# oharari/Convex-Combination-of-Gaussian-Processes

Hardware: AMD Instinct MI355X
Metric: GP log-lik evals/sec (n x n fp64, batched over hyperpar grid) (higher is better)
Workload: dtype f64; 1 GPU; cfg4: synthetic maximin-LHS 5-D design n=4096, K=3 anisotropic components, 512-point hyperparameter grid sharded over the GPUs; n=4096, d=5, K=3, evals_total=512, evals_per_gpu=512, parallelism=grid sharded over 1 GPU(s), one all-gather

## Files before the change

### convex-combination-of-gaussian-processes_amd/api.py

```python
from __future__ import annotations

import ctypes
from ctypes import POINTER, c_char_p, c_double, c_int, c_size_t, c_void_p

import numpy as np

from ._lib import load_library

MEAN_PROFILE_BETA = 0
MEAN_ZERO_PLUS_TAU2 = 1
PRIOR_INVGAMMA, PRIOR_GV, PRIOR_ISO, PRIOR_ANI = 0, 1, 2, 3
T_COV, T_UPDATE, T_DIAG, T_TRSM, T_SOLVE, T_FUSED = range(6)
KERNEL_GAUSS, KERNEL_MATERN, KERNEL_MATERN_SPLINE = 0, 1, 2
OPT_FUSE_DIAG, OPT_TAIL_STRIPS, OPT_WIDE_OFFSETS, OPT_SMALL_GRID16 = 2, 3, 4, 5
OPT_SCHED, OPT_SCHED_POLICY, OPT_PREDICT_FACTOR = 7, 8, 9
TIMING_NAMES = ("cov", "update", "diag", "trsm", "solve", "fused", "sweep")

_dp = POINTER(c_double)
_ip = POINTER(c_int)

SIGNATURES = {
    "ccgp_create": (c_int, [c_int, POINTER(c_void_p)]),
    "ccgp_destroy": (c_int, [c_void_p]),
    "ccgp_last_error": (c_char_p, [c_void_p]),
    "ccgp_version": (c_char_p, []),
    "ccgp_set_stream": (c_int, [c_void_p, c_void_p]),
    "ccgp_set_kernel": (c_int, [c_void_p, c_int, c_double]),
    "ccgp_set_workspace_limit": (c_int, [c_void_p, c_size_t]),
    "ccgp_set_option": (c_int, [c_void_p, c_int, c_int]),
    "ccgp_reserve": (c_int, [c_void_p, c_int, c_int, c_int, c_int, c_int]),
    "ccgp_synchronize": (c_int, [c_void_p]),
    "ccgp_corr_matrix": (c_int, [c_void_p, _dp, c_int, c_int, _dp, _dp]),
    "ccgp_corr_cross": (c_int, [c_void_p, _dp, c_int, _dp, c_int, c_int, _dp, _dp]),
    "ccgp_mixed_corr_matrix": (c_int, [c_void_p, _dp, c_int, c_int, c_int, _dp, _dp]),
    "ccgp_mixed_corr_cross": (c_int, [c_void_p, _dp, c_int, _dp, c_int, c_int, c_int, _dp, _dp]),
    "ccgp_beta_mle": (c_int, [c_void_p, _dp, _dp, c_int, _dp]),
    "ccgp_sigma2_mle": (c_int, [c_void_p, _dp, _dp, c_int, c_double, _dp]),
    "ccgp_loglik_batch": (c_int, [c_void_p, _dp, c_int, c_int, _dp, c_int, _dp, c_int, c_double,
                                  c_int, c_double, _dp, _dp, _ip]),
    "ccgp_loglik_batch_dev": (c_int, [c_void_p, c_void_p, c_int, c_int, c_void_p, c_int, c_void_p,
                                      c_int, c_double, c_int, c_double, c_void_p, c_void_p, c_void_p]),
    "ccgp_loglik_grad_batch": (c_int, [c_void_p, _dp, c_int, c_int, _dp, c_int, _dp, c_int, c_double,
                                       _dp, _dp, _dp, _ip]),
    "ccgp_logpost": (c_int, [c_void_p, _dp, c_int, c_int, _dp, c_double, c_int, _dp, _dp, _dp, _dp,
                             _dp, _dp, _ip]),
    "ccgp_logpost_batch": (c_int, [c_void_p, _dp, c_int, c_int, _dp, c_double, c_int, _dp, c_int, _dp, _dp, _dp, _dp, _ip]),
    "ccgp_grid_marginal": (c_int, [c_void_p, _dp, c_int, c_int, _dp, c_double, _dp, c_int, c_int,
                                   c_double, c_int, c_double, _dp, _ip, _dp]),
# ... 552 lines not shown
```

### convex-combination-of-gaussian-processes_amd/csrc/blocked.hip

```cpp
#include <cstdlib>
#include <vector>

#include "ccgp_internal.h"
#include "sched_logic.h"

namespace ccgp {

typedef double d4 __attribute__((ext_vector_type(4)));

namespace {

__device__ __forceinline__ int tid_now() {
  int t = threadIdx.x;
  asm volatile("" : "+v"(t));
  return t;
}

__device__ __forceinline__ constexpr int swz_src(int l, int parity) { return (((l >> 3) ^ parity) << 4) + ((l & 7) << 1); }

struct GemmArgs {
  double* A;
  size_t a_stride;
  int npad;
  double* invd;
  size_t invd_stride;
  int j, nt, nb;
  int ld;
  int ne;
  int extra_lower;
  int mode;
  double* E;
  size_t e_stride;
  int lde;
  int rows_only;
  int fuse_diag;
  int tail_strips;
  int wide;
  int n_s1;
  int tail_s;
  double* logdet_part;
  int* status;
  int n;
  double ptol;
};

template <int S, bool THIN>
struct TileGeom {
  static constexpr int CW = kTile / S;
  static constexpr int NX = THIN ? (S == 1 ? 2 : 1) : (S == 1 ? 4 : 2);
  static constexpr int NY = THIN ? 1 : (S == 4 ? 2 : 4);
  static constexpr int BK = 16;
  __device__ static int row0(int wave) { return THIN ? 0 : (S == 4 ? wave * 32 : (wave >> 1) * 64); }
  __device__ static int col0(int wave) {
    return THIN ? wave * NX * 16 : (S == 4 ? 0 : (wave & 1) * (S == 1 ? 64 : 32));
  }
};

template <int S, bool THIN, bool TRI>
__device__ __forceinline__ int col_block(int wave, int x) {
  if constexpr (TRI && !THIN) return (wave & 1) + 2 * x;
  else return (TileGeom<S, THIN>::col0(wave) >> 4) + x;
}

template <bool IL>
struct AccMap {
  int row0, col0, l15, l4;
  __device__ __forceinline__ AccMap() {
    const int lane = tid_now() & 63, wave = tid_now() >> 6;
    row0 = TileGeom<1, false>::row0(wave); col0 = TileGeom<1, false>::col0(wave); l15 = lane & 15; l4 = lane >> 4;
  }
  __device__ __forceinline__ int row(int y) const { return IL ? row0 + 4 * l15 + y : row0 + 16 * y + l15; }
  __device__ __forceinline__ int col(int x, int r) const { return IL ? col0 + 16 * r + 4 * l4 + x : col0 + 16 * x + l4 + 4 * r; }
  static constexpr __device__ __forceinline__ int dcol(int x, int r) { return IL ? 16 * r + x : 16 * x + 4 * r; }
  __device__ __forceinline__ double* lane_base(double* C, int ld) const {
    return IL ? C + row0 + 4 * l15 + (size_t)(col0 + 4 * l4) * ld : C + row0 + l15 + (size_t)(col0 + l4) * ld;
  }
};

template <int S, bool THIN, bool TRI = false>
__device__ __forceinline__ void gemm_accumulate(double* smem, const double* P, int ldP, const double* Q,
                                                int ldQ, int Kdim,
                                                d4 (&acc)[TileGeom<S, THIN>::NX][TileGeom<S, THIN>::NY]) {
  static_assert(!TRI || S == 1, "the triangular skip is only wired for full-width tiles");
  constexpr int CW = TileGeom<S, THIN>::CW;
  constexpr int NX = TileGeom<S, THIN>::NX;
  constexpr int NY = TileGeom<S, THIN>::NY;
  constexpr int BKs = TileGeom<S, THIN>::BK;
  constexpr int STAGE = BKs * kTile + BKs * CW;
  constexpr int CPI = kTile / CW;
  constexpr int QI = BKs / CPI / 4;
  const int tid = tid_now(), lane = tid & 63, wave = tid >> 6;
  const int row0 = TileGeom<S, THIN>::row0(wave);
  const int col0 = TileGeom<S, THIN>::col0(wave);
  const bool active = !THIN || col0 < CW;
  const int l15 = lane & 15, l4 = lane >> 4;

#pragma unroll
  for (int x = 0; x < NX; ++x)
#pragma unroll
    for (int y = 0; y < NY; ++y) acc[x][y] = d4{0.0, 0.0, 0.0, 0.0};

  const double* pP = P + swz_src(lane, wave & 1) + (size_t)wave * ldP;
  const size_t stepP = (size_t)4 * ldP;
  constexpr int LPC = 64 / CPI;
  const int qcol_in = lane / LPC, ql = lane % LPC;
  const int qpar = CPI == 1 ? (wave & 1) : (qcol_in & 1);
  const double* pQ = Q + swz_src(ql, qpar) + (size_t)(CPI * wave + qcol_in) * ldQ;
  const size_t stepQ = (size_t)(4 * CPI) * ldQ;

  auto issue = [&](int stage) {
    double* Ps_ = smem + stage * STAGE + wave * kTile;
    double* Qs_ = smem + stage * STAGE + BKs * kTile + wave * kTile;
#pragma unroll
    for (int q = 0; q < BKs / 4; ++q)
      __builtin_amdgcn_global_load_lds((const __attribute__((address_space(1))) void*)(pP + q * stepP),
                                       (__attribute__((address_space(3))) void*)(Ps_ + 4 * q * kTile), 16, 0, 0);
#pragma unroll
    for (int q = 0; q < QI; ++q)
      __builtin_amdgcn_global_load_lds((const __attribute__((address_space(1))) void*)(pQ + q * stepQ),
                                       (__attribute__((address_space(3))) void*)(Qs_ + 4 * q * kTile), 16, 0, 0);
    pP += (BKs / 4) * stepP;
    pQ += QI * stepQ;
  };

  static_assert(BKs == 16, "the pipeline below is written for four k-steps per stage");
  double pfA[NY], qfA[NX], pfB[NY], qfB[NX];
  const int sw = l4 & 1;
#define CCGP_LOADF(PF, QF, STG, KK)                                                              \
  do {                                                                                          \
    const double* Ps_ = smem + (STG) * STAGE;                                                   \
    const double* Qs_ = Ps_ + BKs * kTile;                                                      \
    _Pragma("unroll") for (int y = 0; y < NY; ++y)                                              \
        PF[y] = Ps_[((KK) * 4 + l4) * kTile + ((((row0 >> 4) + y) ^ sw) << 4) + l15];           \
    _Pragma("unroll") for (int x = 0; x < NX; ++x)                                              \
        QF[x] = Qs_[((KK) * 4 + l4) * CW + ((col_block<S, THIN, TRI>(wave, x) ^ sw) << 4) + l15]; \
    __builtin_amdgcn_sched_barrier(0);                                                          \
  } while (0)
#define CCGP_MFMAS(PF, QF, KT, X0, X1)                                                           \
  do {                                                                                          \
    if (active) {                                                                               \
      _Pragma("unroll") for (int x = (X0); x < (X1); ++x) {                                     \
        if (TRI && col_block<S, THIN, TRI>(wave, x) * 16 + 15 < (KT) * BKs) continue;           \
        _Pragma("unroll") for (int y = 0; y < NY; ++y)                                          \
            acc[x][y] = __builtin_amdgcn_mfma_f64_16x16x4f64(QF[x], PF[y], acc[x][y], 0, 0, 0); \
      }                                                                                         \
    }                                                                                           \
    __builtin_amdgcn_sched_barrier(0);                                                          \
  } while (0)
  constexpr int XH = NX > 1 ? 1 : NX;

  const int nk = Kdim / BKs;
  issue(0);
  __syncthreads();
  if (nk > 1) issue(1);
  CCGP_LOADF(pfA, qfA, 0, 0);
  for (int kt = 0; kt < nk; ++kt) {
    const int stg = kt & 1;
    CCGP_MFMAS(pfA, qfA, kt, 0, XH);
    CCGP_LOADF(pfB, qfB, stg, 1);
    CCGP_MFMAS(pfA, qfA, kt, XH, NX);
    CCGP_MFMAS(pfB, qfB, kt, 0, XH);
    CCGP_LOADF(pfA, qfA, stg, 2);
    CCGP_MFMAS(pfB, qfB, kt, XH, NX);
    CCGP_MFMAS(pfA, qfA, kt, 0, XH);
    CCGP_LOADF(pfB, qfB, stg, 3);
    CCGP_MFMAS(pfA, qfA, kt, XH, NX);
    if (kt + 1 < nk) {
      __syncthreads();
      if (kt + 2 < nk) issue(stg);
    }
    CCGP_MFMAS(pfB, qfB, kt, 0, XH);
    if (kt + 1 < nk) CCGP_LOADF(pfA, qfA, stg ^ 1, 0);
    CCGP_MFMAS(pfB, qfB, kt, XH, NX);
  }
#undef CCGP_LOADF
#undef CCGP_MFMAS
}



__device__ __forceinline__ bool fits_buffer_offsets(int Kdim, int ld) {
  return ((size_t)Kdim + 32) * (size_t)ld * 8 < 0xFFFF0000ull;
}

__device__ __forceinline__ void tile_accumulate_il(double* smem, const double* P, int ldP, const double* Q,
                                                   int ldQ, int Kdim, d4 (&acc)[4][4]) {
  constexpr int BKs = 16, STAGE = 2 * BKs * kTile;
  typedef double d2 __attribute__((ext_vector_type(2)));
  const int tid = tid_now(), lane = tid & 63;
  const int wave = __builtin_amdgcn_readfirstlane(tid >> 6);
  const int row0 = (wave >> 1) * 64, col0 = (wave & 1) * 64;
  const int l15 = lane & 15, l4 = lane >> 4;
#pragma unroll
  for (int x = 0; x < 4; ++x)
#pragma unroll
    for (int y = 0; y < 4; ++y) acc[x][y] = d4{0.0, 0.0, 0.0, 0.0};

  const __amdgpu_buffer_rsrc_t rP = __builtin_amdgcn_make_buffer_rsrc((void*)P, 0, -1, 0x00020000);
  const __amdgpu_buffer_rsrc_t rQ = __builtin_amdgcn_make_buffer_rsrc((void*)Q, 0, -1, 0x00020000);
  const unsigned lane_b = (unsigned)lane * 16;
  const unsigned stepP = (unsigned)ldP * 32, stepQ = (unsigned)ldQ * 32;
  unsigned oP = (unsigned)wave * (unsigned)ldP * 8, oQ = (unsigned)wave * (unsigned)ldQ * 8;
  auto request = [&](int stage, int r) {
    double* dst = smem + stage * STAGE + (r >> 2) * (BKs * kTile) + (wave + 4 * (r & 3)) * kTile;
    if (r < 4)
      __builtin_amdgcn_raw_ptr_buffer_load_lds(rP, (__attribute__((address_space(3))) void*)dst, 16, lane_b,
// ... 142 lines not shown
  } while (0)
#define CCGP_RMFMAS(PF, QF, X0, X1)                                                              \
  do {                                                                                          \
    _Pragma("unroll") for (int x = (X0); x < (X1); ++x)                                         \
      _Pragma("unroll") for (int y = 0; y < NY; ++y)                                            \
          acc[x][y] = __builtin_amdgcn_mfma_f64_16x16x4f64(QF[x], PF[y], acc[x][y], 0, 0, 0);   \
    __builtin_amdgcn_sched_barrier(0);                                                          \
  } while (0)

  const int nk = Kdim / BKd;
  const int pre = nk < NST ? nk : NST;
  for (int t = 0; t < pre; ++t) issue(t);
  __builtin_amdgcn_sched_barrier(0);
  wait_and_meet(pre - 1);
  CCGP_RLOADF(pfA, qfA, 0, 0);
  for (int kt = 0; kt < nk; ++kt) {
    const int slot = kt & (NST - 1);
    CCGP_RLOADF(pfB, qfB, slot, 1);
    CCGP_RMFMAS(pfA, qfA, 0, 2);
    if (kt + 1 < nk) {
      const int last_issued = kt + NST - 1 < nk - 1 ? kt + NST - 1 : nk - 1;
      wait_and_meet(last_issued - (kt + 1));
      if (kt + NST < nk) issue(slot);
      __builtin_amdgcn_sched_barrier(0);
    }
    CCGP_RMFMAS(pfB, qfB, 0, 1);
    if (kt + 1 < nk) CCGP_RLOADF(pfA, qfA, (kt + 1) & (NST - 1), 0);
    CCGP_RMFMAS(pfB, qfB, 1, 2);
  }
#undef CCGP_RLOADF
#undef CCGP_RMFMAS
}

template <int S, bool THIN, bool TRI = false, bool RING = false>
__device__ __forceinline__ void gemm_tile(double* smem, const double* P, int ldP, const double* Q,
                                          int ldQ, int Kdim, double* C, int ld, int mode) {
  constexpr int NX = TileGeom<S, THIN>::NX;
  constexpr int NY = TileGeom<S, THIN>::NY;
  d4 acc[NX][NY];
  if constexpr (RING) {
    static_assert((S == 2 || S == 4) && !THIN && !TRI, "the four-stage ring exists for half- and quarter-width update strips");
    strip_accumulate_ring<S>(smem, P, ldP, Q, ldQ, Kdim, acc);
  } else {
    gemm_accumulate<S, THIN, TRI>(smem, P, ldP, Q, ldQ, Kdim, acc);
  }
  const int lane = tid_now() & 63, wave = tid_now() >> 6;
  const int row0 = TileGeom<S, THIN>::row0(wave), col0 = TileGeom<S, THIN>::col0(wave);
  const int l15 = lane & 15, l4 = lane >> 4;
  if (THIN && col0 >= TileGeom<S, THIN>::CW) return;
#pragma unroll
  for (int x = 0; x < NX; ++x) {
    double cv[NY][4];
    if (mode == 0) {
#pragma unroll
      for (int y = 0; y < NY; ++y)
#pragma unroll
        for (int r = 0; r < 4; ++r)
          cv[y][r] = C[row0 + y * 16 + l15 + (size_t)(col_block<S, THIN, TRI>(wave, x) * 16 + l4 + 4 * r) * ld];
    }
#pragma unroll
    for (int y = 0; y < NY; ++y)
#pragma unroll
      for (int r = 0; r < 4; ++r) {
        double* p = C + row0 + y * 16 + l15 + (size_t)(col_block<S, THIN, TRI>(wave, x) * 16 + l4 + 4 * r) * ld;
        *p = mode == 0 ? cv[y][r] - acc[x][y][r] : acc[x][y][r];
      }
  }
}


template <int W>
__device__ __forceinline__ void diag_rhs_accumulate(double* smem, const double* Qp, const double* Tp, int ld,
                                                    int Kdim, d4 (&acc)[11]) {
  constexpr int BKs = 16, TR = 16, STAGE = BKs * kTile + BKs * TR;
  constexpr int RA = W, RB = 7 - W;
  constexpr int CBMAX = RA > RB ? RA : RB;
  constexpr bool XTRA = 2 * W + 1 > CBMAX;
  constexpr int NQ = CBMAX + 1 + (XTRA ? 2 : 0);
  constexpr int NR = W < 2 ? 5 : 4;
  auto frag_of = [](int cb) constexpr { return cb <= CBMAX ? cb : CBMAX + 1 + (cb - 2 * W); };
  auto cb_of_frag = [](int f) constexpr { return f <= CBMAX ? f : 2 * W + (f - CBMAX - 1); };
  const int lane = tid_now() & 63, l15 = lane & 15, l4 = lane >> 4, sw = l4 & 1;

  const __amdgpu_buffer_rsrc_t rQ = __builtin_amdgcn_make_buffer_rsrc((void*)Qp, 0, -1, 0x00020000);
  const __amdgpu_buffer_rsrc_t rT = __builtin_amdgcn_make_buffer_rsrc((void*)Tp, 0, -1, 0x00020000);
  const unsigned lane_q = (unsigned)(swz_src(lane, W & 1) * 8);
  const unsigned lane_t = (unsigned)((((lane & 7) << 1) + (size_t)(lane >> 3) * ld) * 8);
  const unsigned stepQ = (unsigned)ld * 32;
  unsigned oQ = (unsigned)W * (unsigned)ld * 8, oT = (unsigned)(8 * W) * (unsigned)ld * 8;
  auto request = [&](int stage, int r) {
    double* St_ = smem + stage * STAGE;
    if (r < 4)
      __builtin_amdgcn_raw_ptr_buffer_load_lds(rQ, (__attribute__((address_space(3))) void*)(St_ + (W + 4 * r) * kTile),
                                               16, lane_q, oQ + (unsigned)r * stepQ, 0, 0);
    else
      __builtin_amdgcn_raw_ptr_buffer_load_lds(rT, (__attribute__((address_space(3))) void*)(St_ + BKs * kTile + W * 8 * TR),
                                               16, lane_t, oT, 0, 0);
  };
  auto advance = [&]() { oQ += 4 * stepQ; oT += (unsigned)BKs * (unsigned)ld * 8; };

// ... 280 lines not shown
  for (int off = 32; off > 0; off >>= 1) lsum += __shfl_down(lsum, off, 64);
  if ((tid & 63) == 0) red[tid >> 6] = lsum;
  __syncthreads();
  if (tid == 0) {
    g.logdet_part[(size_t)b * g.nt + g.j] = bad ? kNaN : (red[0] + red[1] + red[2] + red[3]);
    if (bad && g.status[b] == 0) g.status[b] = g.j * kTile + bad;
  }

  double* W = g.invd + (size_t)b * g.invd_stride + (size_t)g.j * kTile * kTile;
#pragma unroll
  for (int bb = 0; bb < 8; ++bb) {
    const int c = tx + 16 * bb;
    const double dc = bad ? 1.0 : dvec[c];
    const double sq = sqrt(dc), rs = 1.0 / sq;
#pragma unroll
    for (int a = 0; a < 8; ++a) {
      const int r = ty + 16 * a;
      if (a >= bb) {
        double v = r > c ? M[a][bb] * rs : (r == c ? sq : 0.0);
        C[r + (size_t)c * ld] = bad ? kNaN : v;
      }
      double w = 0.0;
      if (bb >= a) w = c >= r ? I[a][bb] * rs : 0.0;
      W[c + (size_t)r * kTile] = bad ? kNaN : w;
    }
  }
}

__global__ __launch_bounds__(256) void diag_kernel(DiagArgs g) {
  __shared__ double lds[kDiagLdsDoubles];
  diag_factor(g, blockIdx.x, lds);
}

__host__ __device__ inline int gemm_units_per_matrix(int mode, int nt, int j, int ne, int S, int rows_only = 0) {
  if (rows_only) return mode == 0 ? ne * S : ne;
  return mode == 0 ? 1 + ((nt - 1 - j) + ne) * S : (nt - j) + ne;
}

template <int MODE, int S>
__device__ __forceinline__ void gemm_unit(const GemmArgs& g, double* smem, int j, int b, int i, int strip, bool ring) {
  const int ld = g.ld;
  double* Ab = g.A + (size_t)b * g.a_stride;
  const bool thin = i == g.nt;
  const int c0 = strip * (ring ? kTile / g.tail_s : kTile / S);

  int k0 = 0;
  if (g.extra_lower && i > g.nt) {
    const int te = i - g.nt - 1;
    if (j < te || (MODE == 0 && j == te)) return;
    k0 = te * kTile;
  }
  double* rowbase = Ab + (size_t)i * kTile;
  int rld = ld;
  if (g.E && i > g.nt) {
    rowbase = g.E + (size_t)b * g.e_stride + (size_t)(i - g.nt - 1) * kTile;
    rld = g.lde;
  }
  const double* P;
  const double* Q;
  int ldP, ldQ, Kdim;
  if (MODE == 0) {
    P = rowbase + (size_t)k0 * rld;
    Q = Ab + (size_t)j * kTile + c0 + (size_t)k0 * ld;
    ldP = rld;
    ldQ = ld;
    Kdim = j * kTile - k0;
  } else {
    P = rowbase + (size_t)j * kTile * rld;
    Q = g.invd + (size_t)b * g.invd_stride + (size_t)j * kTile * kTile + c0;
    ldP = rld;
    ldQ = kTile;
    Kdim = kTile;
  }
  double* C = rowbase + ((size_t)j * kTile + c0) * rld;
  constexpr bool TRI = MODE == 1 && S == 1;
  if constexpr (MODE == 1) {
    if (thin) { gemm_tile<S, true, TRI>(smem, P, ldP, Q, ldQ, Kdim, C, rld, MODE); return; }
  }
  if constexpr (MODE == 0 && S == 1) {
    if (ring) {
      if (g.tail_s == 4) gemm_tile<4, false, false, true>(smem, P, ldP, Q, ldQ, Kdim, C, rld, MODE);
      else gemm_tile<2, false, false, true>(smem, P, ldP, Q, ldQ, Kdim, C, rld, MODE);
      return;
    }
    if (!g.wide && fits_buffer_offsets(Kdim, ldP > ldQ ? ldP : ldQ)) {
      update_tile_il(smem, P, ldP, Q, ldQ, Kdim, C, rld);
      return;
    }
  }
  gemm_tile<S, false, TRI>(smem, P, ldP, Q, ldQ, Kdim, C, rld, MODE);
}

__device__ __forceinline__ void diag_unit(const GemmArgs& g, double* smem, int j, int b) {
  const int ld = g.ld;
  double* Ab = g.A + (size_t)b * g.a_stride;
  diag_rhs_tile(smem, Ab + (size_t)j * kTile, Ab + g.npad, ld, j * kTile,
                Ab + (size_t)j * kTile + (size_t)j * kTile * ld, Ab + g.npad + (size_t)j * kTile * ld, g.wide);
  if (g.fuse_diag) {
    __syncthreads();
    diag_factor(diag_args(g, j), b, smem);
  }
}

template <int MODE, int S>
__device__ __forceinline__ void gemm_dispatch(const GemmArgs& g, double* smem) {
  const int L = blockIdx.x;
  int b, i, strip = 0;
  bool ring = false;
  if (MODE == 0 && !g.rows_only) {
    const int nb8 = (g.nb + 7) & ~7;
    if (L < nb8) {
      if (L < g.nb) diag_unit(g, smem, g.j, L);
      return;
    }
    const int nfull = (g.nt - 1 - g.j) + g.ne;
    const int Lt = L - nb8;
    int u1;
    if (S == 1) {
      if (Lt >= g.n_s1) {
        const int q = Lt - g.n_s1;
        u1 = g.n_s1 + ((q / (8 * g.tail_s)) << 3) + (q & 7);
        strip = (q >> 3) % g.tail_s;
        ring = true;
      } else {
        u1 = Lt;
      }
    } else {
      u1 = ((Lt / (8 * S)) << 3) + (Lt & 7);
      strip = (Lt >> 3) % S;
    }
    const int per_grp = 8 * nfull;
    const int grp = u1 / per_grp, r = u1 % per_grp;
    b = grp * 8 + (r & 7);
    if (b >= g.nb) return;
    i = g.j + 1 + (r >> 3);
    if (i >= g.nt) i += 1;
  } else {
    const int per_grp = 8 * gemm_units_per_matrix(MODE, g.nt, g.j, g.ne, S, g.rows_only);
    const int grp = L / per_grp, r = L % per_grp;
    b = grp * 8 + (r & 7);
    if (b >= g.nb) return;
    const int u = r >> 3;
    if (g.rows_only) {
      strip = MODE == 0 ? u % S : 0;
      i = g.nt + 1 + (MODE == 0 ? u / S : u);
    } else {
      i = g.j + 1 + u;
    }
  }
  gemm_unit<MODE, S>(g, smem, g.j, b, i, strip, ring);
}

#define CCGP_DEFINE_GEMM(NAME, MODE, S, WPS)                                            \
  __global__ __launch_bounds__(256, WPS) void NAME(GemmArgs g) {                        \
    extern __shared__ __attribute__((aligned(16))) double smem[];                       \
    gemm_dispatch<MODE, S>(g, smem);                                                     \
  }
CCGP_DEFINE_GEMM(chol_update_kernel, 0, 1, 2)
CCGP_DEFINE_GEMM(chol_update_s2_kernel, 0, 2, 2)
CCGP_DEFINE_GEMM(chol_trsm_kernel, 1, 1, 2)
#undef CCGP_DEFINE_GEMM

#include "blocked_sched.inc"


static int update_tail(int nb8, int tiles, int quarters, int* ts) {
  const long w1 = (long)nb8 * (1 + tiles), all_tiles = (long)nb8 * tiles;
  const long rem = w1 % 256;
  *ts = 2;
  if (rem == 0 || all_tiles == 0) return 0;
  long tail = rem < all_tiles ? rem : all_tiles;
  if (tail != rem && w1 > 256) return 0;
  if (quarters && w1 > 256 && (rem - tail) + 4 * tail <= 512) { *ts = 4; return (int)tail; }
  if (rem + tail > 256) return 0;
  return (int)tail;
}

static void launch_gemm(hipStream_t s, GemmArgs g, int mode, int S) {
  const int nb8 = round_up(g.nb, 8);
  int units = nb8 * gemm_units_per_matrix(mode, g.nt, g.j, g.ne, S, g.rows_only);
  if (mode == 0 && !g.rows_only) {
    const int tiles = (g.nt - 1 - g.j) + g.ne;
    int ts = 2;
    const int tail = (S == 1 && g.tail_strips) ? update_tail(nb8, tiles, g.tail_strips == 1, &ts) : 0;
    g.n_s1 = nb8 * tiles - tail;
    g.tail_s = ts;
    units = nb8 + (S == 1 ? g.n_s1 + ts * tail : nb8 * tiles * S);
  }
  const dim3 grid(units), block(256);
  if (mode == 0) {
    if (S == 1) hipLaunchKernelGGL(chol_update_kernel, grid, block, gemm_lds_bytes<1>(), s, g);
    else hipLaunchKernelGGL(chol_update_s2_kernel, grid, block, gemm_lds_bytes<2>(), s, g);
  } else {
    hipLaunchKernelGGL(chol_trsm_kernel, grid, block, gemm_lds_bytes<1>(), s, g);
  }
}

struct RhsArgs {
  double* A;
  size_t a_stride;
  int npad, n;
  const double* y;
  int ld;
  int identity;
};

__global__ __launch_bounds__(256) void rhs_rows_kernel(RhsArgs g) {
  const int ld = g.ld;
  double* Ab = g.A + (size_t)blockIdx.y * g.a_stride;
  const int c = blockIdx.x * 16 + (threadIdx.x >> 4);
  const int r = threadIdx.x & 15;
  double v = 0.0;
  if (c < g.n) v = r == 0 ? g.y[c] : (r == 1 ? 1.0 : 0.0);
// ... 440 lines not shown

struct GroupRun {
  ccgp_handle* h;
  hipStream_t s;
  const double* X;
  int n, d;
  const double* y;
  DrawView dv;
  int b0, nb, npad, nt;
  double sigma2;
  int mean_mode;
  double tau2;
  BlockedWs w;
  double* loglik;
  double* beta;
  int* status;
  const BlockedJob* job;
  GemmArgs g{};
  void begin() {
    const BlockedJob* pr = job && job->kind == kJobPredict ? job : nullptr;
    nt = npad / kTile;
    {
      ScopedTimer t(h, CCGP_T_COV, s);
      launch_cov_tiles(s, X, n, d, dv, b0, nb, w.A, w.a_stride, npad, mean_mode, sigma2, tau2, w.ld, w.xpad, w.upad);
      RhsArgs ra{w.A, w.a_stride, npad, n, y, w.ld, job && job->kind >= kJobInverse ? 1 : 0};
      hipLaunchKernelGGL(rhs_rows_kernel, dim3(npad / 16, nb), dim3(256), 0, s, ra);
      if (pr)
        launch_cov_cross_batched(s, pr->Xtest, pr->m, X, n, d, dv, b0, nb, w.A + npad + kTile, w.a_stride,
                                 w.ld);
    }
    g.A = w.A; g.a_stride = w.a_stride; g.npad = npad; g.invd = w.invd;
    g.invd_stride = (size_t)nt * kTile * kTile; g.nt = nt; g.nb = nb; g.ld = w.ld; g.ne = w.ne;
    g.extra_lower = job && job->kind >= kJobInverse ? 1 : 0;
    g.fuse_diag = h->opt_fuse_diag; g.tail_strips = h->opt_tail_strips; g.wide = h->opt_wide_offsets; g.logdet_part = w.z; g.status = status + b0; g.n = n;
    g.ptol = pivot_tolerance(mean_mode, n);
  }

  void update(int j) {
    if (j == 0) return;
    ScopedTimer t(h, CCGP_T_UPDATE, s);
    g.j = j;
    g.mode = 0;
    launch_gemm(s, g, 0, 1);
  }

  void panel(int j) {
    if (j == 0 || !g.fuse_diag) {
      ScopedTimer t(h, CCGP_T_DIAG, s);
      hipLaunchKernelGGL(diag_kernel, dim3(nb), dim3(256), 0, s, diag_args(g, j));
    }
    {
      ScopedTimer t(h, CCGP_T_TRSM, s);
      g.j = j;
      g.mode = 1;
      launch_gemm(s, g, 1, 1);
    }
  }

  void finish() {
    const BlockedJob* pr = job && job->kind == kJobPredict ? job : nullptr;
    {
      ScopedTimer t(h, CCGP_T_SOLVE, s);
      FinishArgs fa{};
      fa.A = w.A; fa.a_stride = w.a_stride; fa.npad = npad; fa.logdet_part = w.z; fa.params = dv.params;
      fa.ldp = dv.ldp; fa.K = dv.K; fa.b0 = b0; fa.nt = nt; fa.n = n; fa.sigma2 = sigma2;
      fa.mode = mean_mode; fa.loglik = loglik; fa.beta = beta; fa.status = status; fa.ld = w.ld;
      fa.s11_out = w.fin; fa.beta_out = w.fin + nb;
// ... 151 lines not shown
```

### convex-combination-of-gaussian-processes_amd/csrc/capi.hip

```cpp
#include <algorithm>
#include <cmath>
#include <cstdio>
#include <cstdlib>
#include <cstring>
#include <exception>
#include <initializer_list>
#include <map>
#include <memory>
#include <new>
#include <vector>

#include "ccgp_internal.h"
#include "special_math.h"
#include "stage_layout.h"

using namespace ccgp;

namespace {

#define CCGP_HIP(call)                                                              \
  do {                                                                              \
    hipError_t e_ = (call);                                                         \
    if (e_ != hipSuccess) {                                                         \
      h->err = std::string(#call) + ": " + hipGetErrorString(e_);                   \
// ... 612 lines not shown

int ccgp_set_kernel(ccgp_handle* h, int family, double nu) try {
  if (!h) return CCGP_EINVAL;
  if (family == CCGP_KERNEL_GAUSS) {
    h->fam = ccgp::KernelFamily{};
    return CCGP_OK;
  }
  if ((family != CCGP_KERNEL_MATERN && family != CCGP_KERNEL_MATERN_SPLINE) || !(nu > 1.0) || !(nu <= 10.0))
    return fail(h, CCGP_EINVAL, "ccgp_set_kernel: family must be CCGP_KERNEL_GAUSS, or CCGP_KERNEL_MATERN / CCGP_KERNEL_MATERN_SPLINE with 1 < nu <= 10 (the range the quadrature is validated on; the scripts use 5)");
  h->fam.id = family;
  h->fam.nu = nu;
  h->fam.norm = 1.0 / (std::tgamma(nu) * std::pow(2.0, nu - 1.0));
  return CCGP_OK;
} CCGP_GUARD_END(h)

int ccgp_set_workspace_limit(ccgp_handle* h, size_t bytes) try {
  if (!h || bytes < (size_t(1) << 20)) return CCGP_EINVAL;
  h->ws_limit = bytes;
  return CCGP_OK;
} CCGP_GUARD_END(h)

int ccgp_set_option(ccgp_handle* h, int option, int value) try {
  if (!h) return CCGP_EINVAL;
  if (option == CCGP_OPT_TAIL_STRIPS && value >= 0 && value <= 2) {
    h->opt_tail_strips = value;
    return CCGP_OK;
  }
  if (option == CCGP_OPT_FUSE_DIAG && (value == 0 || value == 1)) {
    h->opt_fuse_diag = value;
    return CCGP_OK;
  }
  if (option == CCGP_OPT_WIDE_OFFSETS && (value == 0 || value == 1)) {
    h->opt_wide_offsets = value;
    return CCGP_OK;
  }
  if (option == CCGP_OPT_SMALL_GRID16 && (value == 0 || value == 1)) {
    h->opt_small_grid16 = value;
    return CCGP_OK;
  }
  if (option == CCGP_OPT_PREDICT_FACTOR && (value == 0 || value == 1)) {
    h->opt_predict_factor = value;
    return CCGP_OK;
  }
  if (option == CCGP_OPT_SCHED && value >= 0 && value <= 3) {
    h->opt_sched = value;
    return CCGP_OK;
  }
  if (option == CCGP_OPT_SCHED_POLICY && value >= 0 && value <= 31) {
    h->opt_sched_policy = value;
    return CCGP_OK;
  }
  return fail(h, CCGP_EINVAL, "ccgp_set_option: unknown option or value");
} CCGP_GUARD_END(h)

int ccgp_synchronize(ccgp_handle* h) try {
  if (!h) return CCGP_EINVAL;
  CCGP_HIP(hipStreamSynchronize(h->stream));
  return CCGP_OK;
} CCGP_GUARD_END(h)

int ccgp_reserve(ccgp_handle* h, int n, int d, int K, int B, int m) try {
  if (!h || bad_shape(n, d, K) || B < 1 || m < 0) return fail(h, CCGP_EINVAL, "ccgp_reserve: bad argument");
  CCGP_HIP(hipSetDevice(h->device));
  const bool gauss = h->fam.id == 0;
  const bool sweep_predict = m > 0 && small_route(Op::Predict, gauss, n, d, K) == Route::Blocked;
  if (sweep_predict || small_route(Op::Loglik, gauss, n, d, K) == Route::Blocked) {
// ... 931 lines not shown
```

### convex-combination-of-gaussian-processes_amd/csrc/ccgp_internal.h

```cpp
#pragma once

#include <hip/hip_runtime.h>

#include <cstddef>
#include <atomic>
#include <cstdint>
#include <mutex>
#include <string>
#include <vector>

#include "../../include/ccgp.h"
#include "exp_table.h"
#include "small_layout.h"

namespace ccgp {

constexpr int kTile = 128;

constexpr double kSolvePivotEps = 2.220446049250313e-16;
__host__ __device__ inline double pivot_tolerance(int mean_mode, int n) { return mean_mode == 0 ? n * kSolvePivotEps : 0.0; }

}

namespace ccgp {

struct TimedSpan {
  int id;
  hipEvent_t e0, e1;
};

struct KernelFamily {
  int id = 0;
  double nu = 0.0;
  double norm = 0.0;
};

}

namespace ccgp {
constexpr int kPullSlices = 4;
}

struct ccgp_handle {
  int device = 0;
  hipStream_t own_stream = nullptr;
  hipStream_t stream = nullptr;
  size_t ws_limit = size_t(24) << 30;
  int opt_small_grid16 = 0;
  int opt_predict_factor = 1;
  int opt_fuse_diag = 1;
  int opt_tail_strips = 1;
  int opt_wide_offsets = 0;
  int opt_sched = 3;
  int opt_sched_policy = 11;
  int sched_timeout_ms = 30000;
  int sched_backlog_min = 0;
  int n_cus = 256;
  unsigned long long* sched_prof_dev = nullptr;
  int sched_prof_wgs = 0;
  void* ws = nullptr;
  size_t ws_bytes = 0;
  void* stage = nullptr;
  size_t stage_bytes = 0;
  void* pin = nullptr;
  size_t pin_bytes = 0;
  size_t pin_in = 0;
  hipStream_t aux_stream = nullptr;
  hipEvent_t aux_fork = nullptr, aux_join = nullptr;
  hipEvent_t pull_ev[ccgp::kPullSlices] = {};
  std::string err;
  ccgp::KernelFamily fam;
  unsigned timing = 0;
  std::vector<ccgp::TimedSpan> spans;
  size_t spans_used = 0;
};

namespace ccgp {

struct DrawView {
  const double* params;
  int ldp;
  int K;
  int d;
  KernelFamily fam;
};
// ... 278 lines not shown
```

### include/ccgp.h

```cpp
#ifndef CCGP_H
#define CCGP_H

#include <stddef.h>
#include <stdint.h>

#ifdef __cplusplus
extern "C" {
#endif

typedef struct ccgp_handle ccgp_handle;

enum {
  CCGP_OK = 0,
  CCGP_EINVAL = -1,
  CCGP_EHIP = -2,
  CCGP_ENOMEM = -3,
  CCGP_EUNSUPPORTED = -4
};

enum {
  CCGP_MEAN_PROFILE_BETA = 0,
  CCGP_MEAN_ZERO_PLUS_TAU2 = 1
};

enum {
  CCGP_PRIOR_INVGAMMA = 0,
  CCGP_PRIOR_GV = 1,
  CCGP_PRIOR_ISO = 2,
  CCGP_PRIOR_ANI = 3
};

int ccgp_create(int device, ccgp_handle** out);
int ccgp_destroy(ccgp_handle* h);
const char* ccgp_last_error(const ccgp_handle* h);
const char* ccgp_version(void);
int ccgp_set_stream(ccgp_handle* h, void* hip_stream);
enum { CCGP_KERNEL_GAUSS = 0, CCGP_KERNEL_MATERN = 1, CCGP_KERNEL_MATERN_SPLINE = 2 };
int ccgp_set_kernel(ccgp_handle* h, int family, double nu);
int ccgp_set_workspace_limit(ccgp_handle* h, size_t bytes);
enum { CCGP_OPT_FUSE_DIAG = 2, CCGP_OPT_TAIL_STRIPS = 3, CCGP_OPT_WIDE_OFFSETS = 4, CCGP_OPT_SMALL_GRID16 = 5,
       CCGP_OPT_SCHED = 7, CCGP_OPT_SCHED_POLICY = 8, CCGP_OPT_PREDICT_FACTOR = 9 };
int ccgp_set_option(ccgp_handle* h, int option, int value);
int ccgp_reserve(ccgp_handle* h, int n, int d, int K, int B, int m);
int ccgp_synchronize(ccgp_handle* h);

int ccgp_corr_matrix(ccgp_handle* h, const double* X, int n, int d, const double* theta,
                     double* out_R);
int ccgp_corr_cross(ccgp_handle* h, const double* Xnew, int m, const double* X, int n, int d,
                    const double* theta, double* out);

int ccgp_mixed_corr_matrix(ccgp_handle* h, const double* X, int n, int d, int K,
                           const double* params, double* out_R);
int ccgp_mixed_corr_cross(ccgp_handle* h, const double* Xnew, int m, const double* X, int n,
                          int d, int K, const double* params, double* out);

int ccgp_beta_mle(ccgp_handle* h, const double* R_inv, const double* y, int n, double* out_beta);
int ccgp_sigma2_mle(ccgp_handle* h, const double* R_inv, const double* y, int n, double beta,
                    double* out_sigma2);

int ccgp_loglik_batch(ccgp_handle* h, const double* X, int n, int d, const double* y, int K,
                      const double* params, int B, double sigma2, int mean_mode, double tau2,
                      double* out_loglik, double* out_beta, int* status);
int ccgp_loglik_batch_dev(ccgp_handle* h, const double* dX, int n, int d, const double* dy, int K,
                          const double* dparams, int B, double sigma2, int mean_mode, double tau2,
                          double* d_loglik, double* d_beta, int* d_status);

int ccgp_loglik_grad_batch(ccgp_handle* h, const double* X, int n, int d, const double* y, int K,
                           const double* params, int B, double sigma2, double* out_loglik,
                           double* out_beta, double* out_grad, int* status);

int ccgp_logpost(ccgp_handle* h, const double* X, int n, int d, const double* y, double sigma2,
                 int prior_id, const double* theta_t, const double* prior_pars, double* out_val,
                 double* out_beta, double* out_loglik, double* out_Rinv, int* status);
int ccgp_logpost_batch(ccgp_handle* h, const double* X, int n, int d, const double* y, double sigma2, int prior_id,
// ... 91 lines not shown
```

Measured before the change: 2653 evals/s.

## Pair panel-solve tiles per workgroup, streaming two output tiles through one pipeline

In the blocked Cholesky panel solve (mode 1), each workgroup now handles two vertically adjacent output tiles instead of one. It streams their K-loops back to back through the same double-buffered LDS pipeline, storing the first tile at a seam callback and then resetting the accumulators. This halves the number of trsm workgroups, amortises pipeline fill/drain and the shared Q operand setup, and keeps the prefetch running across the tile boundary. In exchange there is less parallelism per launch, longer per-workgroup latency, and a new default-on option that changes the unit indexing.

```diff
diff --git a/convex-combination-of-gaussian-processes_amd/api.py b/convex-combination-of-gaussian-processes_amd/api.py
--- a/convex-combination-of-gaussian-processes_amd/api.py
+++ b/convex-combination-of-gaussian-processes_amd/api.py
@@ -13,7 +13,7 @@
 T_COV, T_UPDATE, T_DIAG, T_TRSM, T_SOLVE, T_FUSED = range(6)
 KERNEL_GAUSS, KERNEL_MATERN, KERNEL_MATERN_SPLINE = 0, 1, 2
 OPT_FUSE_DIAG, OPT_TAIL_STRIPS, OPT_WIDE_OFFSETS, OPT_SMALL_GRID16 = 2, 3, 4, 5
-OPT_SCHED, OPT_SCHED_POLICY, OPT_PREDICT_FACTOR = 7, 8, 9
+OPT_SCHED, OPT_SCHED_POLICY, OPT_PREDICT_FACTOR, OPT_TRSM_PAIR = 7, 8, 9, 10
 TIMING_NAMES = ("cov", "update", "diag", "trsm", "solve", "fused", "sweep")
 
 _dp = POINTER(c_double)
diff --git a/convex-combination-of-gaussian-processes_amd/csrc/blocked.hip b/convex-combination-of-gaussian-processes_amd/csrc/blocked.hip
--- a/convex-combination-of-gaussian-processes_amd/csrc/blocked.hip
+++ b/convex-combination-of-gaussian-processes_amd/csrc/blocked.hip
@@ -42,6 +42,7 @@
   int* status;
   int n;
   double ptol;
+  int trsm_pair;
 };
 
 template <int S, bool THIN>
@@ -77,11 +78,14 @@
   }
 };
 
-template <int S, bool THIN, bool TRI = false>
+struct NoSeam {};
+template <int S, bool THIN, bool TRI = false, class SEAM = NoSeam>
 __device__ __forceinline__ void gemm_accumulate(double* smem, const double* P, int ldP, const double* Q,
                                                 int ldQ, int Kdim,
-                                                d4 (&acc)[TileGeom<S, THIN>::NX][TileGeom<S, THIN>::NY]) {
+                                                d4 (&acc)[TileGeom<S, THIN>::NX][TileGeom<S, THIN>::NY],
+                                                int ntile = 1, ptrdiff_t tile_step = 0, SEAM seam = SEAM{}) {
   static_assert(!TRI || S == 1, "the triangular skip is only wired for full-width tiles");
+  constexpr bool STREAM = !__is_same(SEAM, NoSeam);
   constexpr int CW = TileGeom<S, THIN>::CW;
   constexpr int NX = TileGeom<S, THIN>::NX;
   constexpr int NY = TileGeom<S, THIN>::NY;
@@ -108,6 +112,8 @@
   const double* pQ = Q + swz_src(ql, qpar) + (size_t)(CPI * wave + qcol_in) * ldQ;
   const size_t stepQ = (size_t)(4 * CPI) * ldQ;
 
+  const int nk = Kdim / BKs;
+  int issued = 0;
   auto issue = [&](int stage) {
     double* Ps_ = smem + stage * STAGE + wave * kTile;
     double* Qs_ = smem + stage * STAGE + BKs * kTile + wave * kTile;
@@ -121,6 +127,13 @@
                                        (__attribute__((address_space(3))) void*)(Qs_ + 4 * q * kTile), 16, 0, 0);
     pP += (BKs / 4) * stepP;
     pQ += QI * stepQ;
+    if constexpr (STREAM) {
+      if (++issued == nk) {
+        issued = 0;
+        pP += tile_step - (ptrdiff_t)Kdim * ldP;
+        pQ -= (ptrdiff_t)Kdim * ldQ;
+      }
+    }
   };
 
   static_assert(BKs == 16, "the pipeline below is written for four k-steps per stage");
@@ -149,29 +162,40 @@
   } while (0)
   constexpr int XH = NX > 1 ? 1 : NX;
 
-  const int nk = Kdim / BKs;
   issue(0);
   __syncthreads();
   if (nk > 1) issue(1);
   CCGP_LOADF(pfA, qfA, 0, 0);
-  for (int kt = 0; kt < nk; ++kt) {
-    const int stg = kt & 1;
-    CCGP_MFMAS(pfA, qfA, kt, 0, XH);
-    CCGP_LOADF(pfB, qfB, stg, 1);
-    CCGP_MFMAS(pfA, qfA, kt, XH, NX);
-    CCGP_MFMAS(pfB, qfB, kt, 0, XH);
-    CCGP_LOADF(pfA, qfA, stg, 2);
-    CCGP_MFMAS(pfB, qfB, kt, XH, NX);
-    CCGP_MFMAS(pfA, qfA, kt, 0, XH);
-    CCGP_LOADF(pfB, qfB, stg, 3);
-    CCGP_MFMAS(pfA, qfA, kt, XH, NX);
-    if (kt + 1 < nk) {
-      __syncthreads();
-      if (kt + 2 < nk) issue(stg);
-    }
-    CCGP_MFMAS(pfB, qfB, kt, 0, XH);
-    if (kt + 1 < nk) CCGP_LOADF(pfA, qfA, stg ^ 1, 0);
-    CCGP_MFMAS(pfB, qfB, kt, XH, NX);
+  for (int t = 0; t < (STREAM ? ntile : 1); ++t) {
+    const bool more = STREAM && t + 1 < ntile;
+    for (int kt = 0; kt < nk; ++kt) {
+      const int stg = kt & 1;
+      CCGP_MFMAS(pfA, qfA, kt, 0, XH);
+      CCGP_LOADF(pfB, qfB, stg, 1);
+      CCGP_MFMAS(pfA, qfA, kt, XH, NX);
+      CCGP_MFMAS(pfB, qfB, kt, 0, XH);
+      CCGP_LOADF(pfA, qfA, stg, 2);
+      CCGP_MFMAS(pfB, qfB, kt, XH, NX);
+      CCGP_MFMAS(pfA, qfA, kt, 0, XH);
+      CCGP_LOADF(pfB, qfB, stg, 3);
+      CCGP_MFMAS(pfA, qfA, kt, XH, NX);
+      if (kt + 1 < nk || more) {
+        __syncthreads();
+        if (kt + 2 < nk || more) issue(stg);
+      }
+      CCGP_MFMAS(pfB, qfB, kt, 0, XH);
+      if (kt + 1 < nk || more) CCGP_LOADF(pfA, qfA, stg ^ 1, 0);
+      CCGP_MFMAS(pfB, qfB, kt, XH, NX);
+    }
+    if constexpr (STREAM) {
+      if (more) {
+        seam(t);
+#pragma unroll
+        for (int x = 0; x < NX; ++x)
+#pragma unroll
+          for (int y = 0; y < NY; ++y) acc[x][y] = d4{0.0, 0.0, 0.0, 0.0};
+      }
+    }
   }
 #undef CCGP_LOADF
 #undef CCGP_MFMAS
@@ -380,40 +404,48 @@
 #undef CCGP_RMFMAS
 }
 
-template <int S, bool THIN, bool TRI = false, bool RING = false>
+template <int S, bool THIN, bool TRI = false, bool RING = false, bool STREAM = false>
 __device__ __forceinline__ void gemm_tile(double* smem, const double* P, int ldP, const double* Q,
-                                          int ldQ, int Kdim, double* C, int ld, int mode) {
+                                          int ldQ, int Kdim, double* C, int ld, int mode, int ntile = 1,
+                                          ptrdiff_t tile_step = 0) {
   constexpr int NX = TileGeom<S, THIN>::NX;
   constexpr int NY = TileGeom<S, THIN>::NY;
   d4 acc[NX][NY];
+  auto store = [&](double* Ct) {
+    const int lane = tid_now() & 63, wave = tid_now() >> 6;
+    const int row0 = TileGeom<S, THIN>::row0(wave), col0 = TileGeom<S, THIN>::col0(wave);
+    const int l15 = lane & 15, l4 = lane >> 4;
+    if (THIN && col0 >= TileGeom<S, THIN>::CW) return;
+#pragma unroll
+    for (int x = 0; x < NX; ++x) {
+      double cv[NY][4];
+      if (mode == 0) {
+#pragma unroll
+        for (int y = 0; y < NY; ++y)
+#pragma unroll
+          for (int r = 0; r < 4; ++r)
+            cv[y][r] = Ct[row0 + y * 16 + l15 + (size_t)(col_block<S, THIN, TRI>(wave, x) * 16 + l4 + 4 * r) * ld];
+      }
+#pragma unroll
+      for (int y = 0; y < NY; ++y)
+#pragma unroll
+        for (int r = 0; r < 4; ++r) {
+          double* p = Ct + row0 + y * 16 + l15 + (size_t)(col_block<S, THIN, TRI>(wave, x) * 16 + l4 + 4 * r) * ld;
+          *p = mode == 0 ? cv[y][r] - acc[x][y][r] : acc[x][y][r];
+        }
+    }
+  };
   if constexpr (RING) {
     static_assert((S == 2 || S == 4) && !THIN && !TRI, "the four-stage ring exists for half- and quarter-width update strips");
     strip_accumulate_ring<S>(smem, P, ldP, Q, ldQ, Kdim, acc);
+  } else if constexpr (STREAM) {
+    gemm_accumulate<S, THIN, TRI>(smem, P, ldP, Q, ldQ, Kdim, acc, ntile, tile_step,
+                                  [&](int t) { store(C + t * tile_step); });
+    C += (ntile - 1) * tile_step;
   } else {
     gemm_accumulate<S, THIN, TRI>(smem, P, ldP, Q, ldQ, Kdim, acc);
   }
-  const int lane = tid_now() & 63, wave = tid_now() >> 6;
-  const int row0 = TileGeom<S, THIN>::row0(wave), col0 = TileGeom<S, THIN>::col0(wave);
-  const int l15 = lane & 15, l4 = lane >> 4;
-  if (THIN && col0 >= TileGeom<S, THIN>::CW) return;
-#pragma unroll
-  for (int x = 0; x < NX; ++x) {
-    double cv[NY][4];
-    if (mode == 0) {
-#pragma unroll
-      for (int y = 0; y < NY; ++y)
-#pragma unroll
-        for (int r = 0; r < 4; ++r)
-          cv[y][r] = C[row0 + y * 16 + l15 + (size_t)(col_block<S, THIN, TRI>(wave, x) * 16 + l4 + 4 * r) * ld];
-    }
-#pragma unroll
-    for (int y = 0; y < NY; ++y)
-#pragma unroll
-      for (int r = 0; r < 4; ++r) {
-        double* p = C + row0 + y * 16 + l15 + (size_t)(col_block<S, THIN, TRI>(wave, x) * 16 + l4 + 4 * r) * ld;
-        *p = mode == 0 ? cv[y][r] - acc[x][y][r] : acc[x][y][r];
-      }
-  }
+  store(C);
 }
 
 
@@ -760,13 +792,16 @@
   diag_factor(g, blockIdx.x, lds);
 }
 
-__host__ __device__ inline int gemm_units_per_matrix(int mode, int nt, int j, int ne, int S, int rows_only = 0) {
+__host__ __device__ inline int gemm_units_per_matrix(int mode, int nt, int j, int ne, int S, int rows_only = 0, int pair = 0) {
   if (rows_only) return mode == 0 ? ne * S : ne;
+  if (mode == 1 && pair) return ((nt - 1 - j) + ne + 1) / 2 + 1;
   return mode == 0 ? 1 + ((nt - 1 - j) + ne) * S : (nt - j) + ne;
 }
 
-template <int MODE, int S>
-__device__ __forceinline__ void gemm_unit(const GemmArgs& g, double* smem, int j, int b, int i, int strip, bool ring) {
+template <int MODE, int S, bool STREAM = false>
+__device__ __forceinline__ void gemm_unit(const GemmArgs& g, double* smem, int j, int b, int i, int strip, bool ring,
+                                          int i2 = -1) {
+  static_assert(!STREAM || (MODE == 1 && S == 1), "only the panel solve streams tiles");
   const int ld = g.ld;
   double* Ab = g.A + (size_t)b * g.a_stride;
   const bool thin = i == g.nt;
@@ -816,6 +851,12 @@
       return;
     }
   }
+  if constexpr (STREAM) {
+    const bool two = i2 >= 0 && !(g.extra_lower && i2 > g.nt && j < i2 - g.nt - 1);
+    gemm_tile<S, false, TRI, false, true>(smem, P, ldP, Q, ldQ, Kdim, C, rld, MODE, two ? 2 : 1,
+                                          (ptrdiff_t)(i2 - i) * kTile);
+    return;
+  }
   gemm_tile<S, false, TRI>(smem, P, ldP, Q, ldQ, Kdim, C, rld, MODE);
 }
 
@@ -833,7 +874,7 @@
 template <int MODE, int S>
 __device__ __forceinline__ void gemm_dispatch(const GemmArgs& g, double* smem) {
   const int L = blockIdx.x;
-  int b, i, strip = 0;
+  int b, i, i2 = -1, strip = 0;
   bool ring = false;
   if (MODE == 0 && !g.rows_only) {
     const int nb8 = (g.nb + 7) & ~7;
@@ -864,7 +905,7 @@
     i = g.j + 1 + (r >> 3);
     if (i >= g.nt) i += 1;
   } else {
-    const int per_grp = 8 * gemm_units_per_matrix(MODE, g.nt, g.j, g.ne, S, g.rows_only);
+    const int per_grp = 8 * gemm_units_per_matrix(MODE, g.nt, g.j, g.ne, S, g.rows_only, g.trsm_pair);
     const int grp = L / per_grp, r = L % per_grp;
     b = grp * 8 + (r & 7);
     if (b >= g.nb) return;
@@ -872,11 +913,20 @@
     if (g.rows_only) {
       strip = MODE == 0 ? u % S : 0;
       i = g.nt + 1 + (MODE == 0 ? u / S : u);
+    } else if (MODE == 1 && g.trsm_pair) {
+      const int nfull = (g.nt - 1 - g.j) + g.ne;
+      auto tile_row = [&](int f) { return g.j + 1 + f + (g.j + 1 + f >= g.nt ? 1 : 0); };
+      if (2 * u >= nfull) {
+        i = g.nt;
+      } else {
+        i = tile_row(2 * u);
+        if (2 * u + 1 < nfull) i2 = tile_row(2 * u + 1);
+      }
     } else {
       i = g.j + 1 + u;
     }
   }
-  gemm_unit<MODE, S>(g, smem, g.j, b, i, strip, ring);
+  gemm_unit<MODE, S, MODE == 1>(g, smem, g.j, b, i, strip, ring, i2);
 }
 
 #define CCGP_DEFINE_GEMM(NAME, MODE, S, WPS)                                            \
@@ -906,7 +956,7 @@
 
 static void launch_gemm(hipStream_t s, GemmArgs g, int mode, int S) {
   const int nb8 = round_up(g.nb, 8);
-  int units = nb8 * gemm_units_per_matrix(mode, g.nt, g.j, g.ne, S, g.rows_only);
+  int units = nb8 * gemm_units_per_matrix(mode, g.nt, g.j, g.ne, S, g.rows_only, g.trsm_pair);
   if (mode == 0 && !g.rows_only) {
     const int tiles = (g.nt - 1 - g.j) + g.ne;
     int ts = 2;
@@ -1413,7 +1463,7 @@
     g.A = w.A; g.a_stride = w.a_stride; g.npad = npad; g.invd = w.invd;
     g.invd_stride = (size_t)nt * kTile * kTile; g.nt = nt; g.nb = nb; g.ld = w.ld; g.ne = w.ne;
     g.extra_lower = job && job->kind >= kJobInverse ? 1 : 0;
-    g.fuse_diag = h->opt_fuse_diag; g.tail_strips = h->opt_tail_strips; g.wide = h->opt_wide_offsets; g.logdet_part = w.z; g.status = status + b0; g.n = n;
+    g.fuse_diag = h->opt_fuse_diag; g.tail_strips = h->opt_tail_strips; g.wide = h->opt_wide_offsets; g.trsm_pair = h->opt_trsm_pair; g.logdet_part = w.z; g.status = status + b0; g.n = n;
     g.ptol = pivot_tolerance(mean_mode, n);
   }
 
diff --git a/convex-combination-of-gaussian-processes_amd/csrc/capi.hip b/convex-combination-of-gaussian-processes_amd/csrc/capi.hip
--- a/convex-combination-of-gaussian-processes_amd/csrc/capi.hip
+++ b/convex-combination-of-gaussian-processes_amd/csrc/capi.hip
@@ -668,6 +668,10 @@
   }
   if (option == CCGP_OPT_WIDE_OFFSETS && (value == 0 || value == 1)) {
     h->opt_wide_offsets = value;
+    return CCGP_OK;
+  }
+  if (option == CCGP_OPT_TRSM_PAIR && (value == 0 || value == 1)) {
+    h->opt_trsm_pair = value;
     return CCGP_OK;
   }
   if (option == CCGP_OPT_SMALL_GRID16 && (value == 0 || value == 1)) {
diff --git a/convex-combination-of-gaussian-processes_amd/csrc/ccgp_internal.h b/convex-combination-of-gaussian-processes_amd/csrc/ccgp_internal.h
--- a/convex-combination-of-gaussian-processes_amd/csrc/ccgp_internal.h
+++ b/convex-combination-of-gaussian-processes_amd/csrc/ccgp_internal.h
@@ -51,6 +51,7 @@
   int opt_fuse_diag = 1;
   int opt_tail_strips = 1;
   int opt_wide_offsets = 0;
+  int opt_trsm_pair = 1;
   int opt_sched = 3;
   int opt_sched_policy = 11;
   int sched_timeout_ms = 30000;
diff --git a/include/ccgp.h b/include/ccgp.h
--- a/include/ccgp.h
+++ b/include/ccgp.h
@@ -39,7 +39,7 @@
 int ccgp_set_kernel(ccgp_handle* h, int family, double nu);
 int ccgp_set_workspace_limit(ccgp_handle* h, size_t bytes);
 enum { CCGP_OPT_FUSE_DIAG = 2, CCGP_OPT_TAIL_STRIPS = 3, CCGP_OPT_WIDE_OFFSETS = 4, CCGP_OPT_SMALL_GRID16 = 5,
-       CCGP_OPT_SCHED = 7, CCGP_OPT_SCHED_POLICY = 8, CCGP_OPT_PREDICT_FACTOR = 9 };
+       CCGP_OPT_SCHED = 7, CCGP_OPT_SCHED_POLICY = 8, CCGP_OPT_PREDICT_FACTOR = 9, CCGP_OPT_TRSM_PAIR = 10 };
 int ccgp_set_option(ccgp_handle* h, int option, int value);
 int ccgp_reserve(ccgp_handle* h, int n, int d, int K, int B, int m);
 int ccgp_synchronize(ccgp_handle* h);
```

After: 2653 evals/s. About the same (-0.0%).
